# hanmekim/SceneLib2

Measured on NVIDIA H100. Metric: EKF-SLAM frames/sec @320x240 N=100 feats, higher is better.
Workload: dtype f64 (EKF, scores) + u8/int32 (correlation sums)

## Files before the change

### scenelib2_b200/csrc/update.cu

```cuda
#include <type_traits>

#include "sl2_context.cuh"
#include "sl2_ptx.cuh"

using namespace sl2;

namespace {

constexpr int UPD_THREADS = 256;
constexpr int UPD_NB = 16;
constexpr int UPD_WS = 20;
constexpr int UPD_DS = 20;
constexpr int UPD_MS = 20;
constexpr int UPD_YS = 68;
constexpr int SOLVE_MAX_WARPS = 8;

__host__ __device__ inline int upd_keven(int kmax) { return (kmax + 1) & ~1; }
__host__ __device__ inline int upd_panw(int kmax) {
  return ((2 * upd_keven(kmax) + 15) & ~15) + 2;
}
__host__ __device__ inline size_t upd_pan_doubles(int kmax) { return (size_t)UPD_NB * upd_panw(kmax); }

__device__ __forceinline__ void dmma884(double &c0, double &c1, double a, double b) {
  asm("mma.sync.aligned.m8n8k4.row.col.f64.f64.f64.f64 {%0,%1}, {%2}, {%3}, {%0,%1};"
// ... 416 lines not shown
    for (int q = 0; q < GB; ++q) dmma1684(c[q], a, bu[q]);
  };
#pragma unroll
  for (int u = 0; u < D - 1; ++u)
    if (u < nk) loadb(b[u]);
  int kb = 0;
  for (; kb + D <= nk; kb += D) {
#pragma unroll
    for (int u = 0; u < D; ++u) {
      if (kb + u + D - 1 < nk) loadb(b[(u + D - 1) % D]);
      step(b[u]);
    }
  }
  if (D == 8 && kb < nk) {
#pragma unroll
    for (int u = 0; u < 4; ++u) step(b[u]);
  }
#pragma unroll
  for (int q = 0; q < GB; ++q) {
    if (g0 + q < ngroups) {
      const int pc = (g0 + q) * 8 + 2 * lc;
#pragma unroll
      for (int mt = 0; mt < 2; ++mt)
        *reinterpret_cast<double2 *>(pan + (size_t)(mt * 8 + lr) * PW + pc) = make_double2(c[q][2 * mt], c[q][2 * mt + 1]);
    }
  }
}

struct CholSmem {
  double *mult;
  double *dpre;
  int msz;
  double *dg;
  double *Wm;
  double *pan;
  int panw;
};
__host__ __device__ inline size_t chol_smem_doubles(int kmax) {
  const size_t mmax = 2 * upd_keven(kmax);
  return 2 * mmax * UPD_MS + 2 * UPD_NB * CH_DPS + UPD_NB * UPD_DS + UPD_NB * UPD_WS + upd_pan_doubles(kmax);
}
__device__ __forceinline__ CholSmem chol_carve(uint8_t *base, int kmax) {
  CholSmem u;
  const int mmax = 2 * upd_keven(kmax);
  double *p = reinterpret_cast<double *>(base);
  u.msz = mmax * UPD_MS;
  u.mult = p;  p += (size_t)2 * u.msz;
  u.dpre = p;  p += 2 * UPD_NB * CH_DPS;
  u.dg = p;  p += UPD_NB * UPD_DS;
  u.Wm = p;  p += UPD_NB * UPD_WS;
  u.pan = p;
  u.panw = upd_panw(kmax);
  return u;
}

__global__ void __launch_bounds__(UPD_THREADS, 2) upd_chol_kernel(const Sl2Dev d, int stream_lo) {
  extern __shared__ __align__(16) uint8_t smem_raw[];
  pdl_prologue();
  const CholSmem sm = chol_carve(smem_raw, d.kmax);
  const int s = stream_lo + blockIdx.x;
  const int tid = threadIdx.x;
  const int ldg = d.ldg;
  double *__restrict__ G = d.G + (size_t)s * d.mmax * ldg;
  double *__restrict__ Wp = d.Wp + (size_t)s * SL2_MAX_PANELS * 256;
  const int warp = tid >> 5, lane = tid & 31;
  const int lr = lane >> 2, lc = lane & 3;
  __shared__ int s_next;
  const int m = d.upd_m[s];
  if (m == 0) return;
  const int width = m;
  const int PW = sm.panw;
  if (tid == 0) s_next = 1;
  __syncthreads();

  for (int i0 = 0, pidx = 0; i0 < m; i0 += UPD_NB, ++pidx) {
    const int par = pidx & 1;
    const double *__restrict__ mcur = sm.mult + par * sm.msz;
    double *__restrict__ mnext = sm.mult + (par ^ 1) * sm.msz;
    const double *__restrict__ dcur = sm.dpre + par * (UPD_NB * CH_DPS);
    double *__restrict__ dnext = sm.dpre + (par ^ 1) * (UPD_NB * CH_DPS);
    const int nbp = min(UPD_NB, m - i0);
    const int n0 = i0 + UPD_NB;
    const int nbn = n0 < m ? min(UPD_NB, m - n0) : 0;
    const int ngroups = (width - i0 + 7) >> 3;
    const int nk = i0 >> 2;
    const int gb = 4;
    const int nbatch = ngroups > 2 ? (ngroups - 2 + gb - 1) / gb : 0;
    const int nitems = 2 + nbatch;
    bool first = true;
    for (;;) {
      int it;
      if (warp == 0 && first) {
        it = 0;
      } else {
        if (lane == 0) it = atomicAdd(&s_next, 1);
        it = __shfl_sync(0xffffffffu, it, 0);
      }
      if (it >= nitems) break;
      if (it == 0) {
        first = false;
        double c[2][4];
        if (pidx == 0) {
#pragma unroll
          for (int q = 0; q < 2; ++q)
#pragma unroll
            for (int mt = 0; mt < 2; ++mt) {
              const int r = mt * 8 + lr, cc = 8 * q + 2 * lc;
              c[q][2 * mt] = (r < nbp && cc < width) ? G[(size_t)r * ldg + cc] : 0.0;
              c[q][2 * mt + 1] = (r < nbp && cc + 1 < width) ? G[(size_t)r * ldg + cc + 1] : 0.0;
            }
        } else {
#pragma unroll
          for (int q = 0; q < 2; ++q)
#pragma unroll
            for (int mt = 0; mt < 2; ++mt) {
              const double2 v = *reinterpret_cast<const double2 *>(dcur + (mt * 8 + lr) * CH_DPS + 8 * q + 2 * lc);
              c[q][2 * mt] = v.x;
              c[q][2 * mt + 1] = v.y;
            }
#pragma unroll
          for (int u = 0; u < 4; ++u) {
            const int st = nk - 4 + u;
            const double a[2] = {mcur[(4 * st + lc) * UPD_MS + lr], mcur[(4 * st + lc) * UPD_MS + 8 + lr]};
            dmma1684(c[0], a, -a[0]);
            dmma1684(c[1], a, -a[1]);
          }
        }
        {
          double *dg = sm.dg;
#pragma unroll
          for (int q = 0; q < 2; ++q)
#pragma unroll
            for (int mt = 0; mt < 2; ++mt) {
              const int r = mt * 8 + lr, cc = 8 * q + 2 * lc;
              const bool rv = r < nbp;
              *reinterpret_cast<double2 *>(dg + r * UPD_DS + cc) =
                  make_double2((rv && cc < nbp) ? c[q][2 * mt] : (r == cc ? 1.0 : 0.0),
                               (rv && cc + 1 < nbp) ? c[q][2 * mt + 1] : (r == cc + 1 ? 1.0 : 0.0));
            }
          sm.Wm[(lane >> 3) * UPD_WS + 8 + (lane & 7)] = 0.0;
          sm.Wm[(4 + (lane >> 3)) * UPD_WS + 8 + (lane & 7)] = 0.0;
          __syncwarp();
          chol8_inv(dg, sm.Wm, 0, lane);
          __syncwarp();
          {
            double c0 = 0.0, c1 = 0.0;
#pragma unroll
            for (int ks = 0; ks < 2; ++ks)
              dmma884(c0, c1, sm.Wm[lr * UPD_WS + 4 * ks + lc], dg[(4 * ks + lc) * UPD_DS + 8 + lr]);
            __syncwarp();
            *reinterpret_cast<double2 *>(dg + lr * UPD_DS + 8 + 2 * lc) = make_double2(c0, c1);
          }
          __syncwarp();
          {
            double2 cv = *reinterpret_cast<const double2 *>(dg + (8 + lr) * UPD_DS + 8 + 2 * lc);
#pragma unroll
            for (int ks = 0; ks < 2; ++ks) {
              const double v = dg[(4 * ks + lc) * UPD_DS + 8 + lr];
              dmma884(cv.x, cv.y, -v, v);
            }
            *reinterpret_cast<double2 *>(dg + (8 + lr) * UPD_DS + 8 + 2 * lc) = cv;
          }
          __syncwarp();
          chol8_inv(dg, sm.Wm, 8, lane);
          __syncwarp();
          {
            double t0 = 0.0, t1 = 0.0;
#pragma unroll
            for (int ks = 0; ks < 2; ++ks)
              dmma884(t0, t1, dg[(4 * ks + lc) * UPD_DS + 8 + lr], sm.Wm[(4 * ks + lc) * UPD_WS + lr]);
            *reinterpret_cast<double2 *>(dg + (8 + lr) * UPD_DS + 2 * lc) = make_double2(t0, t1);
            __syncwarp();
            double w0 = 0.0, w1 = 0.0;
#pragma unroll
            for (int ks = 0; ks < 2; ++ks)
              dmma884(w0, w1, -sm.Wm[(8 + lr) * UPD_WS + 8 + 4 * ks + lc], dg[(8 + 4 * ks + lc) * UPD_DS + lr]);
            *reinterpret_cast<double2 *>(sm.Wm + (8 + lr) * UPD_WS + 2 * lc) = make_double2(w0, w1);
          }
          __syncwarp();
          if (nbp < UPD_NB)
            for (int e = lane; e < UPD_NB * UPD_NB; e += 32) {
              const int i = e >> 4, j = e & 15;
              if (i >= nbp || j >= nbp) sm.Wm[i * UPD_WS + j] = 0.0;
            }
        }
      } else if (it == 1) {
        if (nbn == 0) continue;
        double c[2][4];
#pragma unroll
        for (int q = 0; q < 2; ++q)
#pragma unroll
          for (int mt = 0; mt < 2; ++mt) {
            const int r = mt * 8 + lr, cc = 8 * q + 2 * lc;
            c[q][2 * mt] = (r < nbn && n0 + cc < width) ? G[(size_t)(n0 + r) * ldg + n0 + cc] : 0.0;
            c[q][2 * mt + 1] = (r < nbn && n0 + cc + 1 < width) ? G[(size_t)(n0 + r) * ldg + n0 + cc + 1] : 0.0;
          }
        double v[CH_D][2];
        const size_t kstride = (size_t)4 * ldg;
        const double *gpre = G + (size_t)lc * ldg + n0 + lr;
        double *mp = mnext + lc * UPD_MS + lr;
        const bool v0 = lr < nbn, v1 = 8 + lr < nbn;
        auto loadv = [&](double *dst) {
          const double x0 = gpre[0], x1 = gpre[8];
          dst[0] = v0 ? -x0 : 0.0;
          dst[1] = v1 ? -x1 : 0.0;
          gpre += kstride;
        };
        auto step = [&](const double *vu) {
          const double a[2] = {vu[0], vu[1]};
          mp[0] = a[0];
          mp[8] = a[1];
          mp += 4 * UPD_MS;
          dmma1684(c[0], a, -a[0]);
          dmma1684(c[1], a, -a[1]);
        };
#pragma unroll
        for (int u = 0; u < CH_D - 1; ++u)
          if (u < nk) loadv(v[u]);
        int kb = 0;
        for (; kb + CH_D <= nk; kb += CH_D) {
#pragma unroll
          for (int u = 0; u < CH_D; ++u) {
            if (kb + u + CH_D - 1 < nk) loadv(v[(u + CH_D - 1) % CH_D]);
            step(v[u]);
          }
        }
#pragma unroll
        for (int q = 0; q < 2; ++q)
#pragma unroll
          for (int mt = 0; mt < 2; ++mt)
            *reinterpret_cast<double2 *>(dnext + (mt * 8 + lr) * CH_DPS + 8 * q + 2 * lc) =
                make_double2(c[q][2 * mt], c[q][2 * mt + 1]);
      } else {
        const int bt = it - 2;
        if (gb == 4) chol_batch<4, 4>(G, ldg, mcur, sm.pan, PW, i0, nbp, nk, ngroups, width, 2 + bt * 4, lr, lc);
        else if (gb == 2) chol_batch<2, 8>(G, ldg, mcur, sm.pan, PW, i0, nbp, nk, ngroups, width, 2 + bt * 2, lr, lc);
        else chol_batch<1, 8>(G, ldg, mcur, sm.pan, PW, i0, nbp, nk, ngroups, width, 2 + bt, lr, lc);
      }
    }
    __syncthreads();
    const int ncol = width - i0;
    for (int e = tid; e < UPD_NB * UPD_NB; e += UPD_THREADS) {
      const int r = e / UPD_NB, cc = e - r * UPD_NB;
      if (r < nbp && cc < nbp && i0 + cc < width)
        G[(size_t)(i0 + r) * ldg + i0 + cc] = (cc >= r) ? sm.dg[r * UPD_DS + cc] : 0.0;
      Wp[(size_t)pidx * 256 + e] = sm.Wm[r * UPD_WS + cc];
      if (r >= nbp || UPD_NB + cc >= ncol) mnext[(i0 + r) * UPD_MS + cc] = 0.0;
    }
    if (tid == 0) s_next = 1;
    {
      double aw[4][2];
#pragma unroll
      for (int mt = 0; mt < 2; ++mt)
#pragma unroll
        for (int ks = 0; ks < 4; ++ks) aw[ks][mt] = sm.Wm[(mt * 8 + lr) * UPD_WS + 4 * ks + lc];
      constexpr int FG = 4;
      for (int gb = 2 + warp; gb * 8 < ncol; gb += FG * (UPD_THREADS / 32)) {
        double c[FG][4];
#pragma unroll
        for (int f = 0; f < FG; ++f) c[f][0] = c[f][1] = c[f][2] = c[f][3] = 0.0;
#pragma unroll
        for (int ks = 0; ks < 4; ++ks) {
          double bv[FG];
#pragma unroll
          for (int f = 0; f < FG; ++f) {
            const int cb = (gb + f * (UPD_THREADS / 32)) * 8 + lr;
            bv[f] = cb < ncol ? sm.pan[(size_t)(4 * ks + lc) * PW + cb] : 0.0;
          }
#pragma unroll
          for (int f = 0; f < FG; ++f) dmma1684(c[f], aw[ks], bv[f]);
        }
#pragma unroll
        for (int f = 0; f < FG; ++f) {
          const int gq = gb + f * (UPD_THREADS / 32);
          const int cc = gq * 8 + 2 * lc;
#pragma unroll
          for (int mt = 0; mt < 2; ++mt) {
            const int r = mt * 8 + lr;
            if (r < nbp && cc < ncol) {
              double *dst = G + (size_t)(i0 + r) * ldg + i0 + cc;
              if (cc + 1 < ncol) *reinterpret_cast<double2 *>(dst) = make_double2(c[f][2 * mt], c[f][2 * mt + 1]);
              else *dst = c[f][2 * mt];
              if (gq < 4) {
                mnext[(i0 + r) * UPD_MS + cc - UPD_NB] = -c[f][2 * mt];
                if (cc + 1 < ncol) mnext[(i0 + r) * UPD_MS + cc + 1 - UPD_NB] = -c[f][2 * mt + 1];
              }
            }
          }
        }
      }
    }
    __syncthreads();
  }
}

__device__ __forceinline__ double c_to_b(const double (&c)[2][2], int ks, int lane) {
  const int lr = lane >> 2, lc = lane & 3;
  const int src = ((4 * (ks & 1) + lc) << 2) | (lr >> 1);
  const double v0 = __shfl_sync(0xffffffffu, c[ks >> 1][0], src);
  const double v1 = __shfl_sync(0xffffffffu, c[ks >> 1][1], src);
  return (lr & 1) ? v1 : v0;
}

template <int NP> struct SolveLayout {
  static constexpr int SPLIT = NP > 13 ? 6 : NP;
  static constexpr int REUSE = NP > 13 ? 4 : NP;
  __host__ __device__ static constexpr int pw(int p) { return 16 * (NP - 1 - p) + 4; }
  __host__ __device__ static constexpr int off_lin(int p0, int p) {
    int o = 0;
    for (int q = p0; q < p; ++q) o += 16 * pw(q);
    return o;
  }
  __host__ __device__ static constexpr int off(int p) { return p < SPLIT ? off_lin(0, p) : off_lin(SPLIT, p); }
  static constexpr int PAN_DOUBLES = off_lin(0, SPLIT < NP - 1 ? SPLIT : NP - 1);
  static constexpr int SMEM_DOUBLES = PAN_DOUBLES + NP * 16 * UPD_WS + NP + (NP & 1) +
                                      2 * SOLVE_MAX_WARPS * 2 * 32 * 2 +
                                      SOLVE_MAX_WARPS * 128;
  static_assert(SPLIT == NP || off_lin(SPLIT, NP - 1) <= off_lin(0, REUSE), "second generation must fit");
};

template <int NP>
__global__ void __launch_bounds__(64 * SOLVE_MAX_WARPS, 1) upd_solve_kernel(const Sl2Dev d, int stream_lo) {
  using L = SolveLayout<NP>;
  extern __shared__ __align__(16) uint8_t smem_raw[];
  pdl_prologue();
  double *pan = reinterpret_cast<double *>(smem_raw);
  double *Wm = pan + L::PAN_DOUBLES;
  const uint32_t bars = smem_u32(Wm + NP * 16 * UPD_WS);
  double2 *xbuf = reinterpret_cast<double2 *>(Wm + NP * 16 * UPD_WS + NP + (NP & 1));
  double *ybuf = reinterpret_cast<double *>(xbuf + 2 * SOLVE_MAX_WARPS * 2 * 32);
  const int s = stream_lo + blockIdx.y;
  const int m = d.upd_m[s];
  if (m == 0) return;
  const int tid = threadIdx.x, nthr = blockDim.x;
  const int ngrp = nthr >> 6;
  const int warp = tid >> 5, lane = tid & 31, lr = lane >> 2, lc = lane & 3;
  const int g = warp % ngrp, rho = warp / ngrp;
  const int n = SL2_NXV + 3 * d.nfeat[s];
  const int ncols = n + 1;
  if (blockIdx.x * ngrp * 8 >= ncols) return;
  const int ldg = d.ldg;
  double *__restrict__ G = d.G + (size_t)s * d.mmax * ldg;
  const double *__restrict__ Wp = d.Wp + (size_t)s * SL2_MAX_PANELS * 256;
  const int m8 = (m + 7) & ~7;
  const bool full = L::SPLIT == NP && m8 >= 16 * NP - 8;
  const int zend = full ? 16 * NP : m8;

  if (tid == 0) {
    for (int p = 0; p < NP; ++p) mbar_init(bars + 8 * p, 1);
    fence_barrier_init();
    fence_proxy_async();
  }
  auto zero_pads = [&](int plo, int phi) {
    for (int e = tid; e < (phi - plo) * 16; e += nthr) {
      const int p = plo + (e >> 4), r = e & 15;
      const int cfirst = 16 * p + 16;
      if (16 * p < m)
        for (int c = max(m, cfirst); c < zend; ++c) pan[L::off(p) + r * L::pw(p) + (c - cfirst)] = 0.0;
    }
  };
  zero_pads(0, L::SPLIT);
  __syncthreads();
  auto request = [&](int p) {
    if (16 * p < m) {
      const int cfirst = 16 * p + 16;
      const int nrow = min(16, m - 16 * p);
      const uint32_t ubytes = m > cfirst ? (uint32_t)(m - cfirst) * 8u : 0u;
      const uint32_t bar = bars + 8 * p;
      if (lane == 0) mbar_expect_tx(bar, (uint32_t)nrow * ubytes + 16u * 128u);
      __syncwarp();
      if (lane < 16) {
        if (lane < nrow && ubytes)
          bulk_g2s(pan + L::off(p) + lane * L::pw(p), G + (size_t)(16 * p + lane) * ldg + cfirst, ubytes, bar);
      } else {
        bulk_g2s(Wm + ((size_t)p * 16 + (lane - 16)) * UPD_WS, Wp + (size_t)p * 256 + (lane - 16) * 16, 128u, bar);
      }
    }
  };
  if (warp == 0) {
#pragma unroll 1
    for (int p = 0; p < L::SPLIT; ++p) request(p);
  }

  int xpar = 0;
  auto solve_group = [&](auto full_c, const int grp) {
    constexpr bool FULL = decltype(full_c)::value;
    const int c0 = 8 * grp;
    const bool wact = c0 < ncols;
    const int cc = c0 + 2 * lc;
    const int cval = wact ? min(2, ncols - cc) : 0;
    double *gcol = G + m + cc;
    double acc[(NP + 1) & ~1][2];
    {
      const int ccn = cc + 8 * (int)(gridDim.x * ngrp);
      if (L::SPLIT >= NP && ccn < ncols) {
#pragma unroll
        for (int t = 0; t < NP; ++t) {
          const int row = 8 * (2 * t + rho) + lr;
          if (row < m) asm volatile("prefetch.global.L2 [%0];" ::"l"(G + m + ccn + (size_t)row * ldg));
        }
      }
    }
#pragma unroll
    for (int t = 0; t < ((NP + 1) & ~1); ++t) {
      const int row = 8 * (2 * t + rho) + lr;
      acc[t][0] = acc[t][1] = 0.0;
      if (row < m) {
        if (cval >= 2) {
          const double2 v = *reinterpret_cast<const double2 *>(gcol + (size_t)row * ldg);
          acc[t][0] = v.x;
          acc[t][1] = v.y;
        } else if (cval == 1) {
          acc[t][0] = gcol[(size_t)row * ldg];
        }
      }
    }

#pragma unroll
    for (int p = 0; p < NP; ++p) {
      if (FULL || 16 * p < m) {
        if (L::SPLIT < NP && p == L::REUSE) {
          __syncthreads();
          zero_pads(L::SPLIT, NP);
          __syncthreads();
          if (warp == 0) {
            fence_proxy_async();
#pragma unroll 1
            for (int q = L::SPLIT; q < NP; ++q) request(q);
          }
        }
        if (!wact) continue;
        xpar ^= 1;
        double2 *xb = xbuf + ((size_t)(xpar * ngrp + g) * 2) * 32;
        xb[rho * 32 + lane] = make_double2(acc[p][0], acc[p][1]);
        asm volatile("bar.sync %0, 64;" ::"r"(1 + g) : "memory");
        const double2 other = xb[(rho ^ 1) * 32 + lane];
        const double cp2[2][2] = {{rho ? other.x : acc[p][0], rho ? other.y : acc[p][1]},
                                  {rho ? acc[p][0] : other.x, rho ? acc[p][1] : other.y}};
        mbar_wait(bars + 8 * p, 0);
        const double *pb = pan + L::off(p);
        const int PW = L::pw(p);
        const double *wb = Wm + (size_t)p * 16 * UPD_WS;
        double cb[4];
#pragma unroll
        for (int ks = 0; ks < 4; ++ks) cb[ks] = c_to_b(cp2, ks, lane);
        double d0 = 0.0, d1 = 0.0;
#pragma unroll
        for (int ks = 0; ks < 4; ++ks) dmma884(d0, d1, wb[(8 * rho + lr) * UPD_WS + 4 * ks + lc], cb[ks]);
        {
          const int row = 16 * p + 8 * rho + lr;
          if (row < m) {
            if (cval >= 2) *reinterpret_cast<double2 *>(gcol + (size_t)row * ldg) = make_double2(d0, d1);
            else if (cval == 1) gcol[(size_t)row * ldg] = d0;
          }
        }
        if (p + 1 < NP) {
          double *yg = ybuf + (size_t)g * 128;
          *reinterpret_cast<double2 *>(yg + (8 * rho + lr) * 8 + 2 * lc) = make_double2(d0, d1);
          asm volatile("bar.sync %0, 64;" ::"r"(1 + g) : "memory");
          double yb[4];
#pragma unroll
          for (int ks = 0; ks < 4; ++ks) yb[ks] = -yg[(4 * ks + lc) * 8 + lr];
          const double *pbr = pb + 8 * rho + lr;
#pragma unroll
          for (int ks = 0; ks < 4; ++ks) {
#pragma unroll
            for (int t = (p + 1) & ~1; t < NP; t += 2) {
              const bool has[2] = {t > p && (FULL || 8 * (2 * t + rho) < m),
                                   t + 1 < NP && (FULL || 8 * (2 * t + 2 + rho) < m)};
              if (has[0] || has[1]) {
                double a[2];
#pragma unroll
                for (int h = 0; h < 2; ++h) a[h] = has[h] ? pbr[(4 * ks + lc) * PW + 16 * (t + h - p - 1)] : 0.0;
                double c[4] = {acc[t][0], acc[t][1], acc[t + 1][0], acc[t + 1][1]};
                dmma1684(c, a, yb[ks]);
                acc[t][0] = c[0];
                acc[t][1] = c[1];
                acc[t + 1][0] = c[2];
                acc[t + 1][1] = c[3];
              }
            }
          }
        }
      }
    }
  };
  for (int grp = blockIdx.x * ngrp + g; L::SPLIT < NP ? grp == (int)(blockIdx.x * ngrp + g) : 8 * grp < ncols;
       grp += gridDim.x * ngrp) {
    if (L::SPLIT == NP && full) solve_group(std::true_type{}, grp);
    else solve_group(std::false_type{}, grp);
  }
}

constexpr int SYRK_THREADS = 128;
template <int KC, int ST>
__global__ void __launch_bounds__(SYRK_THREADS, 3) upd_syrk_kernel(const Sl2Dev d, int stream_lo) {
  constexpr int STAGE = 2 * KC * UPD_YS;
  constexpr int NW = SYRK_THREADS / 32;
  extern __shared__ __align__(16) uint8_t smem_raw[];
  double *stage_buf = reinterpret_cast<double *>(smem_raw);
  pdl_prologue();
  const int s = stream_lo + blockIdx.y;
  const int m = d.upd_m[s];
  if (m == 0) return;
  const int n = SL2_NXV + 3 * d.nfeat[s];
  int tb = 0;
  const int t = blockIdx.x;
  while ((tb + 1) * (tb + 2) / 2 <= t) ++tb;
  const int ta = t - tb * (tb + 1) / 2;
  if (tb * 64 >= n + 1) return;
  const int tid = threadIdx.x, warp = tid >> 5, lane = tid & 31, lr = lane >> 2, lc = lane & 3;
  const int wa = (warp & 1) * 32, wb = (warp >> 1) * 32;
  const int ld = d.ld, ldg = d.ldg;
  double *__restrict__ P = d.P + (size_t)s * ld * ld;
  double *__restrict__ x = d.x + (size_t)s * ld;
  const double *__restrict__ G = d.G + (size_t)s * d.mmax * ldg;
  const bool diag = ta == tb;
  const int bi0 = wa >> 3, bj0 = wb >> 3;
  unsigned cmask = 0xFFFFu, mmask = 0xFFFFu;
  if (diag) {
    cmask = mmask = 0u;
#pragma unroll
    for (int bi = 0; bi < 4; ++bi)
#pragma unroll
      for (int bj = 0; bj < 4; ++bj) {
        if (bi0 + bi <= bj0 + bj) cmask |= 1u << (4 * bi + bj);
        if (bi0 + bi < bj0 + bj) mmask |= 1u << (4 * bi + bj);
      }
  }
  const bool skip = cmask == 0u;
  if (!skip) {
#pragma unroll
    for (int i = 0; i < 4; ++i) {
      const int a = ta * 64 + wa + i * 8, bq = tb * 64 + wb + lane;
      if (a < n && bq < n) asm volatile("prefetch.global.L2 [%0];" ::"l"(P + a + (size_t)ld * bq));
    }
  }
  const int kr = m, lim = m + n + 1;
  const int nchunk = (kr + KC - 1) / KC;
  const int cA = m + ta * 64 + 2 * lane, cB = m + tb * 64 + 2 * lane;
  const int bytesA = cA + 1 < lim ? 16 : (cA < lim ? 8 : 0);
  const int bytesB = cB + 1 < lim ? 16 : (cB < lim ? 8 : 0);
  const double *srcA = G + (bytesA ? cA : 0);
  const double *srcB = G + (bytesB ? cB : 0);
  const double *pa = srcA + (size_t)warp * ldg, *pb = srcB + (size_t)warp * ldg;
  const uint32_t sdst = smem_u32(stage_buf + 2 * lane + warp * UPD_YS);
  const size_t rstep = (size_t)NW * ldg;
  auto stage = [&](int chunk) {
    const uint32_t dd = sdst + (uint32_t)(chunk % ST) * (STAGE * 8);
    if ((chunk + 1) * KC <= kr) {
#pragma unroll
      for (int j = 0; j < KC / NW; ++j) {
        asm volatile("cp.async.cg.shared.global [%0], [%1], 16, %2;" ::"r"(dd + j * NW * UPD_YS * 8),
                     "l"(pa + j * rstep), "r"(bytesA)
                     : "memory");
        if (!diag)
          asm volatile("cp.async.cg.shared.global [%0], [%1], 16, %2;" ::"r"(dd + (KC + j * NW) * UPD_YS * 8),
                       "l"(pb + j * rstep), "r"(bytesB)
                       : "memory");
      }
    } else {
#pragma unroll
      for (int j = 0; j < KC / NW; ++j) {
        const bool kv = chunk * KC + warp + NW * j < kr;
        asm volatile("cp.async.cg.shared.global [%0], [%1], 16, %2;" ::"r"(dd + j * NW * UPD_YS * 8),
                     "l"(kv ? pa + j * rstep : srcA), "r"(kv ? bytesA : 0)
                     : "memory");
        if (!diag)
          asm volatile("cp.async.cg.shared.global [%0], [%1], 16, %2;" ::"r"(dd + (KC + j * NW) * UPD_YS * 8),
                       "l"(kv ? pb + j * rstep : srcB), "r"(kv ? bytesB : 0)
                       : "memory");
      }
    }
    pa += (size_t)KC * ldg;
    pb += (size_t)KC * ldg;
  };
  double acc[2][4][4];
#pragma unroll
  for (int i = 0; i < 2; ++i)
#pragma unroll
    for (int j = 0; j < 4; ++j)
#pragma unroll
      for (int e = 0; e < 4; ++e) acc[i][j][e] = 0.0;
#pragma unroll
  for (int c = 0; c < ST - 1; ++c) {
    if (c < nchunk) stage(c);
    cp_async_commit();
  }
  for (int ch = 0; ch < nchunk; ++ch) {
    cp_async_wait<ST - 2>();
    __syncthreads();
    if (ch + ST - 1 < nchunk) stage(ch + ST - 1);
    cp_async_commit();
    if (!skip) {
      const double *Ya = stage_buf + (size_t)(ch % ST) * STAGE;
      const double *Yb = diag ? Ya : Ya + KC * UPD_YS;
      const int krem = kr - ch * KC;
      auto chunk = [&](auto diag_c) {
        constexpr bool DIAG = decltype(diag_c)::value;
        auto kstep = [&](int kk) {
          double a[2][4], b[4][2];
#pragma unroll
          for (int i = 0; i < 2; ++i)
#pragma unroll
            for (int e = 0; e < 4; ++e)
              a[i][e] = Ya[(kk + lc + 4 * (e >> 1)) * UPD_YS + wa + 16 * i + 8 * (e & 1) + lr];
#pragma unroll
          for (int j = 0; j < 4; ++j)
#pragma unroll
            for (int e = 0; e < 2; ++e) b[j][e] = Yb[(kk + lc + 4 * e) * UPD_YS + wb + j * 8 + lr];
#pragma unroll
          for (int i = 0; i < 2; ++i)
#pragma unroll
            for (int j = 0; j < 4; ++j)
              if (!DIAG || 2 * i <= j) dmma1688(acc[i][j], a[i], b[j]);
        };
        if (krem >= KC) {
#pragma unroll
          for (int kk = 0; kk < KC; kk += 8) kstep(kk);
        } else {
#pragma unroll 1
          for (int kk = 0; kk < krem; kk += 8) kstep(kk);
        }
      };
      if (cmask == 0xFFFFu) chunk(std::false_type{});
      else chunk(std::true_type{});
    }
  }
  if (skip) return;
#pragma unroll
  for (int bi = 0; bi < 4; ++bi) {
    const int i = bi >> 1, h = bi & 1;
    const int a = ta * 64 + wa + bi * 8 + lr;
    double pold[4][2];
#pragma unroll
    for (int j = 0; j < 4; ++j)
#pragma unroll
      for (int e = 0; e < 2; ++e) {
        const int bq = tb * 64 + wb + j * 8 + 2 * lc + e;
        pold[j][e] = (((cmask >> (4 * bi + j)) & 1u) && a < n && bq < n) ? P[a + (size_t)ld * bq] : 0.0;
      }
#pragma unroll
    for (int j = 0; j < 4; ++j) {
      if (!((cmask >> (4 * bi + j)) & 1u)) continue;
      const int bq = tb * 64 + wb + j * 8 + 2 * lc;
      const double c0 = acc[i][j][2 * h], c1 = acc[i][j][2 * h + 1];
      const double v0 = pold[j][0] - c0, v1 = pold[j][1] - c1;
      if (a < n && bq < n) {
        P[a + (size_t)ld * bq] = v0;
        if (bq + 1 < n) P[a + (size_t)ld * (bq + 1)] = v1;
        if ((mmask >> (4 * bi + j)) & 1u) {
          double *dst = P + bq + (size_t)ld * a;
          if (bq + 1 < n) *reinterpret_cast<double2 *>(dst) = make_double2(v0, v1);
          else *dst = v0;
        }
      }
      if (a < n) {
        if (bq == n) x[a] += c0;
        if (bq + 1 == n) x[a] += c1;
      }
    }
  }
}

__global__ void __launch_bounds__(UPD_THREADS) upd_finish_kernel(const Sl2Dev d, int stream_lo, int staged,
                                                                  int only_normalise) {
  pdl_prologue();
  const int s = stream_lo + blockIdx.x;
  const int tid = threadIdx.x;
  const int nf = d.nfeat[s];
  const int n = SL2_NXV + 3 * nf;
  const int ld = d.ld;
  double *__restrict__ P = d.P + (size_t)s * ld * ld;
  const double *__restrict__ x = d.x + (size_t)s * ld;
  const size_t fb = (size_t)s * d.Nmax;
  const int m = only_normalise ? 0 : d.upd_m[s];
  __shared__ int s_cull;
  if (m > 0 || only_normalise) {
    __shared__ double J4[16];
    if (tid == 0) {
      const rd q[4] = {rd(x[3]), rd(x[4]), rd(x[5]), rd(x[6])};
      const rd qq = q[0] * q[0] + q[1] * q[1] + q[2] * q[2] + q[3] * q[3];
      for (int i = 0; i < 4; ++i)
        for (int j = 0; j < 4; ++j)
          J4[i * 4 + j] = (i == j) ? ((rd(1.0) - q[i] * q[i] / (qq * qq)) / qq).v
                                   : ((-q[i]) * q[j] / (qq * qq * qq)).v;
    }
    __syncthreads();
    for (int j = tid; j < n; j += UPD_THREADS) {
      double v[4], o[4];
      for (int k = 0; k < 4; ++k) v[k] = P[(3 + k) + (size_t)ld * j];
      for (int i = 0; i < 4; ++i) {
        rd a(0.0);
        for (int k = 0; k < 4; ++k) a = a + rd(J4[i * 4 + k]) * rd(v[k]);
        o[i] = a.v;
      }
      for (int k = 0; k < 4; ++k) P[(3 + k) + (size_t)ld * j] = o[k];
    }
    __syncthreads();
    for (int i = tid; i < n; i += UPD_THREADS) {
      if (i < SL2_NXV) {
        double v[4], o[4];
        for (int k = 0; k < 4; ++k) v[k] = P[i + (size_t)ld * (3 + k)];
        for (int c = 0; c < 4; ++c) {
          rd a(0.0);
          for (int k = 0; k < 4; ++k) a = a + rd(v[k]) * rd(J4[c * 4 + k]);
          o[c] = a.v;
        }
        for (int k = 0; k < 4; ++k) P[i + (size_t)ld * (3 + k)] = o[k];
      } else {
        for (int k = 0; k < 4; ++k) P[i + (size_t)ld * (3 + k)] = P[(3 + k) + (size_t)ld * i];
      }
    }
    __syncthreads();
  }
  {
    const int i = tid % 13, j = (tid / 13) % 13;
    const double a = P[i + (size_t)ld * j], b = P[j + (size_t)ld * i];
    const double v = (rd(a) * rd(0.5) + rd(b) * rd(0.5)).v;
    __syncthreads();
    if (tid < 169) P[i + (size_t)ld * j] = v;
    __syncthreads();
  }
  if (!staged && !only_normalise) {
    if (tid == 0) s_cull = 0;
    __syncthreads();
    for (int i = tid; i < nf; i += UPD_THREADS) {
      int att = d.attempted[fb + i], suc = d.successful[fb + i];
      if (d.sel_rank[fb + i] >= 0) {
        att += 1;
        if (d.found[fb + i] == 1) suc += 1;
        d.attempted[fb + i] = att;
        d.successful[fb + i] = suc;
      }
      if (att >= d.min_attempts && (double)suc / (double)att < d.match_fraction) atomicAdd(&s_cull, 1);
    }
    __syncthreads();
    if (tid == 0) d.ncull[s] = s_cull;
  }
}

struct SolveKernel {
  void (*kern)(Sl2Dev, int);
  int np;
  size_t smem;
};
template <int NP>
SolveKernel solve_kernel_np() {
  return {upd_solve_kernel<NP>, NP, SolveLayout<NP>::SMEM_DOUBLES * sizeof(double)};
}
inline SolveKernel solve_kernel(int kmax) {
  const int p = (2 * upd_keven(kmax) + 15) / 16;
  return p <= 4 ? solve_kernel_np<4>()
                : (p <= 7 ? solve_kernel_np<7>()
                          : (p <= 10 ? solve_kernel_np<10>() : (p <= 13 ? solve_kernel_np<13>() : solve_kernel_np<16>())));
}
inline void solve_shape(int Nmax, int &nslab, int &warps) {
  const int ngroups = (SL2_NXV + 3 * Nmax + 1 + 7) / 8;
  nslab = (ngroups + SOLVE_MAX_WARPS - 1) / SOLVE_MAX_WARPS;
  warps = (ngroups + nslab - 1) / nslab;
}
constexpr size_t SYRK_SMEM = (size_t)2 * 2 * 32 * UPD_YS * sizeof(double);

size_t sl2_update_smem_bytes(const Sl2Dev &d) {
  return chol_smem_doubles(d.kmax) * sizeof(double);
}

}

cudaError_t sl2_configure_update(const Sl2Dev &d) {
  const SolveKernel solve = solve_kernel(d.kmax);
  const struct {
    const void *kern;
    size_t smem;
  } opt_in[] = {
      {(const void *)upd_hp_kernel<7>, hp_layout(d.kmax, d.ld, 0).bytes},
      {(const void *)upd_hp_kernel<13>, hp_layout(d.kmax, d.ld, 0).bytes},
      {(const void *)upd_hp2_kernel<7>, hp_layout(d.kmax, d.ld, 7).bytes},
      {(const void *)upd_hp2_kernel<13>, hp_layout(d.kmax, d.ld, 13).bytes},
      {(const void *)upd_chol_kernel, sl2_update_smem_bytes(d)},
      {(const void *)solve.kern, solve.smem},
      {(const void *)upd_syrk_kernel<32, 2>, SYRK_SMEM},
  };
  for (const auto &k : opt_in) {
    const cudaError_t e = cudaFuncSetAttribute(k.kern, cudaFuncAttributeMaxDynamicSharedMemorySize, (int)k.smem);
    if (e != cudaSuccess) return e;
  }
  return cudaSuccess;
}

cudaError_t sl2_launch_update(const Sl2Dev &d, int stream_lo, int stream_cnt, int staged_m,
                              const int *st_feat, const double *st_Hxv, const double *st_Hy,
                              const double *st_R, const double *st_nu, int only_normalise,
                              Sl2Queue q, cudaEvent_t *ev6) {
// ... 92 lines not shown
```

Before: 233,900.

## Software-pipeline next column group loads into solve loop and drop L2 prefetch

Restructures the triangular solve kernel's column-group loop so each tile of the next group is loaded into registers right after the current group finishes with that tile, instead of issuing L2 prefetches and reloading at the start of each group. Loads now use an ld.global.L2::256B hint. It also adds compile-time-disabled phase instrumentation macros. The aim is to hide global load latency across groups, at the cost of extra live registers and a change in how the loop terminates.

```diff
diff --git a/scenelib2_b200/csrc/update.cu b/scenelib2_b200/csrc/update.cu
--- a/scenelib2_b200/csrc/update.cu
+++ b/scenelib2_b200/csrc/update.cu
@@ -742,6 +742,12 @@
   return (lr & 1) ? v1 : v0;
 }
 
+__device__ __forceinline__ double2 ld_l2_256(const double *p) {
+  double2 v;
+  asm volatile("ld.global.L2::256B.v2.f64 {%0,%1}, [%2];" : "=d"(v.x), "=d"(v.y) : "l"(p));
+  return v;
+}
+
 template <int NP> struct SolveLayout {
   static constexpr int SPLIT = NP > 13 ? 6 : NP;
   static constexpr int REUSE = NP > 13 ? 4 : NP;
@@ -759,10 +765,18 @@
   static_assert(SPLIT == NP || off_lin(SPLIT, NP - 1) <= off_lin(0, REUSE), "second generation must fit");
 };
 
+#ifndef SOLVE_PHASE
+#define SOLVE_PHASE_BEGIN()
+#define SOLVE_PHASE(ph, p, dep)
+#define SOLVE_PHASE_END()
+#endif
+enum { PH_PROLOGUE, PH_ACC, PH_SWAP, PH_MBAR, PH_YP, PH_YSTORE, PH_TRAIL, PH_TAIL };
+
 template <int NP>
 __global__ void __launch_bounds__(64 * SOLVE_MAX_WARPS, 1) upd_solve_kernel(const Sl2Dev d, int stream_lo) {
   using L = SolveLayout<NP>;
   extern __shared__ __align__(16) uint8_t smem_raw[];
+  SOLVE_PHASE_BEGIN();
   pdl_prologue();
   double *pan = reinterpret_cast<double *>(smem_raw);
   double *Wm = pan + L::PAN_DOUBLES;
@@ -821,115 +835,123 @@
 #pragma unroll 1
     for (int p = 0; p < L::SPLIT; ++p) request(p);
   }
+  SOLVE_PHASE(PH_PROLOGUE, 0, 0.0);
 
   int xpar = 0;
-  auto solve_group = [&](auto full_c, const int grp) {
+  const int grp0 = blockIdx.x * ngrp + g, gstep = gridDim.x * ngrp;
+  auto last_group = [&](int grp) { return L::SPLIT < NP || 8 * (grp + gstep) >= ncols; };
+  auto walk = [&](auto full_c) {
     constexpr bool FULL = decltype(full_c)::value;
-    const int c0 = 8 * grp;
-    const bool wact = c0 < ncols;
-    const int cc = c0 + 2 * lc;
-    const int cval = wact ? min(2, ncols - cc) : 0;
-    double *gcol = G + m + cc;
     double acc[(NP + 1) & ~1][2];
-    {
-      const int ccn = cc + 8 * (int)(gridDim.x * ngrp);
-      if (L::SPLIT >= NP && ccn < ncols) {
-#pragma unroll
-        for (int t = 0; t < NP; ++t) {
-          const int row = 8 * (2 * t + rho) + lr;
-          if (row < m) asm volatile("prefetch.global.L2 [%0];" ::"l"(G + m + ccn + (size_t)row * ldg));
-        }
-      }
-    }
-#pragma unroll
-    for (int t = 0; t < ((NP + 1) & ~1); ++t) {
+    auto load_tile = [&](int t, int grp) {
+      const int cc = 8 * grp + 2 * lc;
       const int row = 8 * (2 * t + rho) + lr;
       acc[t][0] = acc[t][1] = 0.0;
       if (row < m) {
-        if (cval >= 2) {
-          const double2 v = *reinterpret_cast<const double2 *>(gcol + (size_t)row * ldg);
+        const double *src = G + m + cc + (size_t)row * ldg;
+        if (cc + 1 < ncols) {
+          const double2 v = ld_l2_256(src);
           acc[t][0] = v.x;
           acc[t][1] = v.y;
-        } else if (cval == 1) {
-          acc[t][0] = gcol[(size_t)row * ldg];
+        } else if (cc < ncols) {
+          acc[t][0] = *src;
         }
       }
-    }
-
-#pragma unroll
-    for (int p = 0; p < NP; ++p) {
-      if (FULL || 16 * p < m) {
-        if (L::SPLIT < NP && p == L::REUSE) {
-          __syncthreads();
-          zero_pads(L::SPLIT, NP);
-          __syncthreads();
-          if (warp == 0) {
-            fence_proxy_async();
+    };
+#pragma unroll
+    for (int t = 0; t < NP; ++t) load_tile(t, grp0);
+    for (int grp = grp0;; grp += gstep) {
+      const int c0 = 8 * grp;
+      const bool wact = c0 < ncols;
+      const int cc = c0 + 2 * lc;
+      const int cval = wact ? min(2, ncols - cc) : 0;
+      double *gcol = G + m + cc;
+      const bool more = !last_group(grp);
+      if constexpr ((NP & 1) != 0) acc[NP][0] = acc[NP][1] = 0.0;
+      SOLVE_PHASE(PH_ACC, min((grp - grp0) / gstep, 15), acc[NP - 1][1]);
+
+#pragma unroll
+      for (int p = 0; p < NP; ++p) {
+        if (FULL || 16 * p < m) {
+          if (L::SPLIT < NP && p == L::REUSE) {
+            __syncthreads();
+            zero_pads(L::SPLIT, NP);
+            __syncthreads();
+            if (warp == 0) {
+              fence_proxy_async();
 #pragma unroll 1
-            for (int q = L::SPLIT; q < NP; ++q) request(q);
+              for (int q = L::SPLIT; q < NP; ++q) request(q);
+            }
+          }
+          if (!wact) continue;
+          xpar ^= 1;
+          double2 *xb = xbuf + ((size_t)(xpar * ngrp + g) * 2) * 32;
+          xb[rho * 32 + lane] = make_double2(acc[p][0], acc[p][1]);
+          asm volatile("bar.sync %0, 64;" ::"r"(1 + g) : "memory");
+          const double2 other = xb[(rho ^ 1) * 32 + lane];
+          const double cp2[2][2] = {{rho ? other.x : acc[p][0], rho ? other.y : acc[p][1]},
+                                    {rho ? acc[p][0] : other.x, rho ? acc[p][1] : other.y}};
+          SOLVE_PHASE(PH_SWAP, p, other.y);
+          mbar_wait(bars + 8 * p, 0);
+          SOLVE_PHASE(PH_MBAR, p, 0.0);
+          const double *pb = pan + L::off(p);
+          const int PW = L::pw(p);
+          const double *wb = Wm + (size_t)p * 16 * UPD_WS;
+          double cb[4];
+#pragma unroll
+          for (int ks = 0; ks < 4; ++ks) cb[ks] = c_to_b(cp2, ks, lane);
+          double d0 = 0.0, d1 = 0.0;
+#pragma unroll
+          for (int ks = 0; ks < 4; ++ks) dmma884(d0, d1, wb[(8 * rho + lr) * UPD_WS + 4 * ks + lc], cb[ks]);
+          SOLVE_PHASE(PH_YP, p, d1);
+          {
+            const int row = 16 * p + 8 * rho + lr;
+            if (row < m) {
+              if (cval >= 2) *reinterpret_cast<double2 *>(gcol + (size_t)row * ldg) = make_double2(d0, d1);
+              else if (cval == 1) gcol[(size_t)row * ldg] = d0;
+            }
+          }
+          if (p + 1 < NP) {
+            double *yg = ybuf + (size_t)g * 128;
+            *reinterpret_cast<double2 *>(yg + (8 * rho + lr) * 8 + 2 * lc) = make_double2(d0, d1);
+            asm volatile("bar.sync %0, 64;" ::"r"(1 + g) : "memory");
+            double yb[4];
+#pragma unroll
+            for (int ks = 0; ks < 4; ++ks) yb[ks] = -yg[(4 * ks + lc) * 8 + lr];
+            SOLVE_PHASE(PH_YSTORE, p, yb[3]);
+            const double *pbr = pb + 8 * rho + lr;
+#pragma unroll
+            for (int ks = 0; ks < 4; ++ks) {
+#pragma unroll
+              for (int t = (p + 1) & ~1; t < NP; t += 2) {
+                const bool has[2] = {t > p && (FULL || 8 * (2 * t + rho) < m),
+                                     t + 1 < NP && (FULL || 8 * (2 * t + 2 + rho) < m)};
+                if (has[0] || has[1]) {
+                  double a[2];
+#pragma unroll
+                  for (int h = 0; h < 2; ++h) a[h] = has[h] ? pbr[(4 * ks + lc) * PW + 16 * (t + h - p - 1)] : 0.0;
+                  double c[4] = {acc[t][0], acc[t][1], acc[t + 1][0], acc[t + 1][1]};
+                  dmma1684(c, a, yb[ks]);
+                  acc[t][0] = c[0];
+                  acc[t][1] = c[1];
+                  acc[t + 1][0] = c[2];
+                  acc[t + 1][1] = c[3];
+                }
+              }
+            }
+            SOLVE_PHASE(PH_TRAIL, p, acc[p + 1][1]);
+          } else {
+            SOLVE_PHASE(PH_YSTORE, p, d1);
           }
         }
-        if (!wact) continue;
-        xpar ^= 1;
-        double2 *xb = xbuf + ((size_t)(xpar * ngrp + g) * 2) * 32;
-        xb[rho * 32 + lane] = make_double2(acc[p][0], acc[p][1]);
-        asm volatile("bar.sync %0, 64;" ::"r"(1 + g) : "memory");
-        const double2 other = xb[(rho ^ 1) * 32 + lane];
-        const double cp2[2][2] = {{rho ? other.x : acc[p][0], rho ? other.y : acc[p][1]},
-                                  {rho ? acc[p][0] : other.x, rho ? acc[p][1] : other.y}};
-        mbar_wait(bars + 8 * p, 0);
-        const double *pb = pan + L::off(p);
-        const int PW = L::pw(p);
-        const double *wb = Wm + (size_t)p * 16 * UPD_WS;
-        double cb[4];
-#pragma unroll
-        for (int ks = 0; ks < 4; ++ks) cb[ks] = c_to_b(cp2, ks, lane);
-        double d0 = 0.0, d1 = 0.0;
-#pragma unroll
-        for (int ks = 0; ks < 4; ++ks) dmma884(d0, d1, wb[(8 * rho + lr) * UPD_WS + 4 * ks + lc], cb[ks]);
-        {
-          const int row = 16 * p + 8 * rho + lr;
-          if (row < m) {
-            if (cval >= 2) *reinterpret_cast<double2 *>(gcol + (size_t)row * ldg) = make_double2(d0, d1);
-            else if (cval == 1) gcol[(size_t)row * ldg] = d0;
-          }
-        }
-        if (p + 1 < NP) {
-          double *yg = ybuf + (size_t)g * 128;
-          *reinterpret_cast<double2 *>(yg + (8 * rho + lr) * 8 + 2 * lc) = make_double2(d0, d1);
-          asm volatile("bar.sync %0, 64;" ::"r"(1 + g) : "memory");
-          double yb[4];
-#pragma unroll
-          for (int ks = 0; ks < 4; ++ks) yb[ks] = -yg[(4 * ks + lc) * 8 + lr];
-          const double *pbr = pb + 8 * rho + lr;
-#pragma unroll
-          for (int ks = 0; ks < 4; ++ks) {
-#pragma unroll
-            for (int t = (p + 1) & ~1; t < NP; t += 2) {
-              const bool has[2] = {t > p && (FULL || 8 * (2 * t + rho) < m),
-                                   t + 1 < NP && (FULL || 8 * (2 * t + 2 + rho) < m)};
-              if (has[0] || has[1]) {
-                double a[2];
-#pragma unroll
-                for (int h = 0; h < 2; ++h) a[h] = has[h] ? pbr[(4 * ks + lc) * PW + 16 * (t + h - p - 1)] : 0.0;
-                double c[4] = {acc[t][0], acc[t][1], acc[t + 1][0], acc[t + 1][1]};
-                dmma1684(c, a, yb[ks]);
-                acc[t][0] = c[0];
-                acc[t][1] = c[1];
-                acc[t + 1][0] = c[2];
-                acc[t + 1][1] = c[3];
-              }
-            }
-          }
-        }
-      }
+        if (more) load_tile(p, grp + gstep);
+      }
+      if (!more) break;
     }
   };
-  for (int grp = blockIdx.x * ngrp + g; L::SPLIT < NP ? grp == (int)(blockIdx.x * ngrp + g) : 8 * grp < ncols;
-       grp += gridDim.x * ngrp) {
-    if (L::SPLIT == NP && full) solve_group(std::true_type{}, grp);
-    else solve_group(std::false_type{}, grp);
-  }
+  if (L::SPLIT == NP && full) walk(std::true_type{});
+  else walk(std::false_type{});
+  SOLVE_PHASE_END();
 }
 
 constexpr int SYRK_THREADS = 128;
```

Result: faster. 237,100, median of 6 (+1.3%).
